# RyanXLi/OneshotDet

Measured on AMD Instinct MI355X. Metric: images/sec/GPU fwd+bwd, 800x1024 target + 127x127 query, bs=8; 1->8 GPU scaling, higher is better.
Workload: dtype bf16; 1 GPU; BASELINE.json configs[2]: bs=8/GPU, 800x1024 target + 127x127 query, bf16 MFMA convs, forward (two R-50-FPN backbones, query pooling, correlation, FCOS head, training proposals) + FCOS loss + backward (stem/layer1 frozen) + gradient all-reduce + SGD(momentum) + weight repack; global_batch=8, parallelism=dp1: one rank, no collective anywhere in the step, world_size=1

## Files before the change

oneshotdet_amd/build.py:

```python
import os
import subprocess
import sys

HERE = os.path.dirname(os.path.abspath(__file__))
CSRC = os.path.join(HERE, "csrc")
LIBDIR = os.path.join(HERE, "lib")
TAG = os.environ.get("OSD_BUILD_TAG", "")
LIB = os.path.join(LIBDIR, "liboneshotdet_hip%s.so" % ("_" + TAG if TAG else ""))
SOURCES = ["osd_error.hip", "conv_igemm.hip", "conv_igemm_dma.hip", "conv_igemm_sp.hip", "conv_pred.hip", "conv_px.hip", "conv_wgrad.hip", "conv_wgrad_sk.hip", "backward.hip", "groupnorm_onepass.hip", "loss.hip", "elementwise.hip", "proposals.hip", "box_head.hip", "transforms.hip", "box_train.hip", "evaluation.hip", "query_avgpool.hip"]
HIPCC = os.environ.get("HIPCC", "/opt/rocm/bin/hipcc")
FLAGS = ["--offload-arch=gfx950", "-O3", "-fPIC", "-std=c++17", "-Wno-unused-result"] + os.environ.get("OSD_BUILD_FLAGS", "").split()


def _stale(target, deps):
    if not os.path.exists(target):
        return True
    t = os.path.getmtime(target)
    return any(os.path.getmtime(d) > t for d in deps)


def build_library(force=False, verbose=True):
    os.makedirs(LIBDIR, exist_ok=True)
    objdir = os.path.join(LIBDIR, "obj" + ("_" + TAG if TAG else ""))
    os.makedirs(objdir, exist_ok=True)
    headers = sorted(os.path.join(CSRC, f) for f in os.listdir(CSRC) if f.endswith(".h")) + [os.path.join(os.path.dirname(HERE), "include", h) for h in ("oneshotdet_hip.h", "oneshotdet_hip_box_modes.h", "oneshotdet_hip_soft_labels.h")]
    keep = set(src.replace(".hip", ".o") for src in SOURCES)
    for f in os.listdir(objdir):
        if f.endswith(".o") and f not in keep:
            os.remove(os.path.join(objdir, f))
    objs, procs = [], []
    for src in SOURCES:
        s = os.path.join(CSRC, src)
        o = os.path.join(objdir, src.replace(".hip", ".o"))
        objs.append(o)
        if force or _stale(o, [s] + headers):
            cmd = [HIPCC] + FLAGS + ["-c", s, "-o", o]
            if verbose:
                print(" ".join(cmd), flush=True)
            procs.append((src, subprocess.Popen(cmd, stdout=subprocess.PIPE, stderr=subprocess.STDOUT)))
    for src, p in procs:
        out, _ = p.communicate()
        if p.returncode != 0:
            sys.stderr.write(out.decode())
            raise RuntimeError("hipcc failed on %s" % src)
    if force or procs or _stale(LIB, objs):
        cmd = [HIPCC, "--offload-arch=gfx950", "-shared", "-fPIC", "-o", LIB] + objs
        if verbose:
            print(" ".join(cmd), flush=True)
        subprocess.check_call(cmd)
    return LIB


if __name__ == "__main__":
    print(build_library(force="--force" in sys.argv))
```

oneshotdet_amd/csrc/conv_wgrad.hip:

```cpp
#include "wgrad_params.h"

namespace {

__device__ __attribute__((aligned(256))) unsigned g_wzero[64];

__device__ __forceinline__ void wg_dma16(const void* gsrc, unsigned lds_dst) {
  unsigned keep;
  asm volatile(
      "s_mov_b32 %0, m0\n\ts_mov_b32 m0, %2\n\ts_nop 0\n\tglobal_load_lds_dwordx4 %1, off\n\ts_mov_b32 m0, %0"
      : "=&s"(keep)
      : "v"(gsrc), "s"(lds_dst)
      : "memory");
}

template <typename T, int BKP, int NST, int WCO, int WCI, int WM, int WN, bool ILV = false>
__global__ void __launch_bounds__(64 * WM * WN, (WM * WN == 4 && WCO + WCI == 3) ? 2 : 1) conv_wgrad_kernel(WgradParams gp) {
  constexpr int NW = WM * WN;
  constexpr int EPC = 16 / (int)sizeof(T);
  constexpr int TWS = 256 / (int)sizeof(T);
  constexpr int TCO = WCO * TWS, TCI = WCI * TWS;
  constexpr int OPB = BKP * 256;
  constexpr int STAGE = (WCO + WCI) * OPB;
  constexpr int PPS = BKP / 4;
  constexpr int IPA = WCO * PPS / NW;
// ... 717 lines not shown
#pragma unroll
          for (int k = 0; k < 4; ++k) red[((co * 9 + t) * 4 + k) * 64 + lane] = acc[co][t][k];
    }
    __syncthreads();
    if (wave == 0) {
#pragma unroll
      for (int co = 0; co < 4; ++co)
#pragma unroll
        for (int t = 0; t < 9; ++t)
#pragma unroll
          for (int k = 0; k < 4; ++k) acc[co][t][k] += red[((co * 9 + t) * 4 + k) * 64 + lane];
    }
    __syncthreads();
  }
  if (wave == 0) {
    float* pp = part + ((size_t)blockIdx.x * gridDim.y + cg) * 36 * 256 + lane * 4;
#pragma unroll
    for (int co = 0; co < 4; ++co)
#pragma unroll
      for (int t = 0; t < 9; ++t)
        *reinterpret_cast<f32x4*>(pp + (co * 9 + t) * 256) = f32x4{acc[co][t][0], acc[co][t][1], acc[co][t][2], acc[co][t][3]};
  }
  if (cg == 0) {
    if (lane == 4) {
#pragma unroll
      for (int co = 0; co < 4; ++co) part_b[((size_t)blockIdx.x * 4 + wave) * 4 + co] = bsum[co];
    }
  }
}

__global__ void pred_wgrad_reduce_kernel(const float* __restrict__ part, const float* __restrict__ part_b, float* __restrict__ dw,
                                         float* __restrict__ db, int blocks, int groups, int C, int cout) {
  const int i = blockIdx.x * blockDim.x + threadIdx.x;
  const int n = cout * 9 * C;
  const int per = (blocks + gridDim.y - 1) / gridDim.y;
  const int b0 = blockIdx.y * per, b1 = min(blocks, b0 + per);
  if (i < n) {
    const int c = i % C, ct = i / C;
    const int cg = c >> 8, cl = c & 255;
    const size_t stride = (size_t)groups * 36 * 256;
    const float* p = part + ((size_t)cg * 36 + ct) * 256 + cl;
    float s0 = 0.f, s1 = 0.f, s2 = 0.f, s3 = 0.f;
    int b = b0;
    for (; b + 3 < b1; b += 4) {
      s0 += p[(size_t)b * stride]; s1 += p[(size_t)(b + 1) * stride]; s2 += p[(size_t)(b + 2) * stride]; s3 += p[(size_t)(b + 3) * stride];
    }
    for (; b < b1; ++b) s0 += p[(size_t)b * stride];
    if (b0 < b1) atomicAdd(dw + i, (s0 + s1) + (s2 + s3));
  } else if (db != nullptr && i < n + cout) {
    const int co = i - n;
    float s = 0.f;
    for (int b = b0 * 4; b < b1 * 4; ++b) s += part_b[(size_t)b * 4 + co];
    if (b0 < b1) atomicAdd(db + co, s);
  }
}

template <typename T>
__global__ void __launch_bounds__(256) bias_grad_kernel(const T* __restrict__ dy, float* __restrict__ db, int M, int C,
                                                        int stride, int rows_per_block) {
  const int c = blockIdx.y * blockDim.x + threadIdx.x;
  const int p_lo = blockIdx.x * rows_per_block, p_hi = min(M, p_lo + rows_per_block);
  if (c >= C || p_lo >= p_hi) return;
  float s = 0.f;
  for (int m = p_lo; m < p_hi; ++m) s += to_f32(dy[(size_t)m * stride + c]);
  atomicAdd(db + c, s);
}

}

#define OSD_STREAM(s) reinterpret_cast<hipStream_t>(s)

extern "C" int osd_bias_grad(const void* dy, float* db, int m, int c, int stride, int dtype, void* stream);

static bool wgrad_dense_input(const osd_conv_desc* d) {
  return d->in_stride_w == d->cin && d->in_stride_h == d->w * d->cin && (long long)d->in_stride_n == (long long)d->h * d->w * d->cin;
}

struct WgradProblem {
  const osd_conv_desc* d;
  int n, h, w;
  const void* x; const void* dy; const float* scale; float* dw; float* db;
};

static int wgrad_xr_launch(int n_seg, const WgradProblem* pr, hipStream_t s) {
  if (n_seg < 1 || n_seg > kMaxSeg) return osd_fail(OSD_ERR_INVALID_ARG, "wgrad: 1..%d segments", kMaxSeg);
  const osd_conv_desc* d0 = pr[0].d;
  static const int kTargets[8] = {512, 256, 128, 64, 1024, 768, 1536, 2048};
  const int a = d0->algo - 1 - 128;
  const int x = a & 15, target = kTargets[(a >> 4) & 7];
  if (a < 0 || a >= 128 || x > 2) return osd_fail(OSD_ERR_INVALID_ARG, "wgrad: unknown algo %d", d0->algo);
  const int bkp = x == 1 ? 64 : 32;
  WgradParams p;
  p.n_seg = n_seg;
  p.sk_units = 0;
  long long work = 0;
  for (int i = 0; i < n_seg; ++i) {
    const osd_conv_desc* d = pr[i].d;
    WgradSeg& g = p.seg[i];
    g.owner = 0;
    const int h = pr[i].h, w = pr[i].w;
    if (d->dtype != OSD_BF16 || d->r != 3 || d->s != 3 || d->stride_h != 1 || d->stride_w != 1 || d->pad_h != 1 || d->pad_w != 1 ||
        d->cout % 128 || d->cin % 128 || d->out_stride % 8 || !(w % bkp == 0 || bkp % w == 0))
      return osd_fail(OSD_ERR_UNSUPPORTED, "wgrad (filter-row kernel): bf16 3x3 / 1 / 1, channels in 128s, width %d vs %d-pixel stages", w, bkp);
    const long long M = (long long)pr[i].n * h * w;
    if (M <= 0 || M > 0x7fffffffLL || !pr[i].x || !pr[i].dy || !pr[i].dw) return osd_fail(OSD_ERR_INVALID_ARG, "wgrad: bad segment %d", i);
    if (M * d->cin > 0x7fffffffLL) return osd_fail(OSD_ERR_UNSUPPORTED, "wgrad: input of segment %d has more than 2^31 elements", i);
    g.x = pr[i].x; g.dy = pr[i].dy; g.dw = pr[i].dw; g.scale = pr[i].scale; g.db = pr[i].db;
    g.H = h; g.W = w; g.Ho = h; g.Wo = w; g.M = (int)M;
    g.Cin = d->cin; g.Cout = d->cout; g.R = 3; g.S = 3; g.sh = g.sw = 1; g.ph = g.pw = 1;
    g.dy_stride = d->out_stride; g.Ktot = 9 * d->cin;
    g.tilesCo = d->cout / 128; g.tilesCi = d->cin / 128;
    work += M * g.tilesCo * g.tilesCi * 3;
  }
  long long rows = (work + target - 1) / target;
  rows = (rows + 63) / 64 * 64;
  if (rows < 128) rows = 128;
  long long nblocks = 0;
  for (int i = 0; i < n_seg; ++i) {
    WgradSeg& g = p.seg[i];
    int sp = (int)((g.M + rows - 1) / rows);
    if (sp < 1) sp = 1;
    g.rows_per_split = cdiv(cdiv(g.M, sp), 64) * 64;
    const int splits = cdiv(g.M, g.rows_per_split);
    g.block_begin = (int)nblocks;
    nblocks += (long long)g.tilesCo * g.tilesCi * 3 * splits;
    if (nblocks > 0x7fffffffLL) return osd_fail(OSD_ERR_INVALID_ARG, "wgrad: bad grid");
  }
  for (int i = n_seg; i < kMaxSeg; ++i) p.seg[i] = p.seg[0];
  p.n_blocks = (int)nblocks;
  p.partials = nullptr;
#define OSD_WGX(BK, NS)                                                                                               \
  do {                                                                                                                \
    auto kern = conv_wgrad_xr_kernel<BK, NS>;                                                                         \
    constexpr int lds = NS * (BK + BK + 4) * 256;                                                                     \
    static bool attr = false;                                                                                         \
    if (!attr) { (void)hipFuncSetAttribute(reinterpret_cast<const void*>(kern), hipFuncAttributeMaxDynamicSharedMemorySize, lds); attr = true; } \
    hipLaunchKernelGGL(kern, dim3((unsigned)nblocks), dim3(512), lds, s, p);                                         \
  } while (0)
  if (x == 0) OSD_WGX(32, 6);
  else if (x == 1) OSD_WGX(64, 4);
  else OSD_WGX(32, 8);
#undef OSD_WGX
  return osd_check_launch("conv_wgrad_xr");
}

static int wgrad_launch_v(int n_seg, const WgradProblem* pr, hipStream_t s, int variant_override);
static int wgrad_launch(int n_seg, const WgradProblem* pr, hipStream_t s) {
  int rc = wgrad_launch_v(n_seg, pr, s, -1);
  if (rc == OSD_ERR_UNSUPPORTED && n_seg >= 1 && pr[0].d->algo == 0) rc = wgrad_launch_v(n_seg, pr, s, 0);
  return rc;
}

static int wgrad_launch_v(int n_seg, const WgradProblem* pr, hipStream_t s, int variant_override) {
  if (n_seg < 1 || n_seg > kMaxSeg) return osd_fail(OSD_ERR_INVALID_ARG, "wgrad: 1..%d segments", kMaxSeg);
  const osd_conv_desc* d0 = pr[0].d;
  if (d0->algo > 128) return wgrad_xr_launch(n_seg, pr, s);
  static int env_target = -1, env_variant = -1;
  if (env_target < 0) { const char* e = getenv("OSD_WGRAD_BLOCKS"); env_target = e ? atoi(e) : 512; }
  if (env_variant < 0) { const char* e = getenv("OSD_WGRAD_VARIANT"); env_variant = e ? atoi(e) : 0; }
  static const int kTargets[8] = {512, 256, 128, 64, 1024, 768, 1536, 2048};
  int target = env_target, variant = variant_override >= 0 ? variant_override : env_variant, code = 0;
  if (d0->algo > 0) {
    const int a = d0->algo - 1;
    if (a >= 128) return osd_fail(OSD_ERR_INVALID_ARG, "wgrad: unknown algo %d", d0->algo);
    variant = a & 15;
    code = a >> 4;
    target = kTargets[code];
  }
  if (d0->dtype == OSD_F32) target *= 8;
  const bool bf = d0->dtype == OSD_BF16;
  if (!bf && variant != 0) variant = 0;
  const int sub_co = bf && (variant == 3 || variant == 4 || variant == 5 || variant == 7 || variant == 8 || variant == 9 || variant == 11 || variant == 13 || variant == 14) ? 2 : 1;
// ... 459 lines not shown
```

oneshotdet_amd/csrc/wgrad_params.h:

```cpp
#pragma once
#include "osd_common.h"
#include <cstddef>

constexpr int kMaxSeg = 24;

struct WgradSeg {
  const void* x;
  const void* dy;
  float* dw;
  const float* scale;
  float* db;
  int H, W, Ho, Wo, M, rows_per_split;
  int Cin, Cout, R, S, sh, sw, ph, pw, dy_stride, tilesCo, tilesCi, Ktot;
  int block_begin;
  int stage_begin;
  int owner;
};

struct WgradParams {
  WgradSeg seg[kMaxSeg];
  int n_seg;
  int n_blocks;
  int sk_units;
  int sk_teams;
  int sk_total;
  float* partials;
};

typedef __attribute__((address_space(1))) float wg_gfloat;
__device__ __forceinline__ void wg_atomic_add(float* ptr, float v) {
  (void)__hip_atomic_fetch_add((wg_gfloat*)ptr, v, __ATOMIC_RELAXED, __HIP_MEMORY_SCOPE_AGENT);
}

template <int TA, int TB>
__device__ __forceinline__ void wg_owner_add(float* base, int Ktot, const f32x4 (&acc)[TA][TB], const float (&scv)[TA][4]) {
#pragma unroll
  for (int i = 0; i < TA; ++i) {
    float old[4][TB];
#pragma unroll
    for (int e = 0; e < 4; ++e)
#pragma unroll
      for (int j = 0; j < TB; ++j) old[e][j] = ((const wg_gfloat*)(base + (size_t)(i * 16 + e) * Ktot))[j * 16];
#pragma unroll
    for (int e = 0; e < 4; ++e)
#pragma unroll
      for (int j = 0; j < TB; ++j) ((wg_gfloat*)(base + (size_t)(i * 16 + e) * Ktot))[j * 16] = old[e][j] + acc[i][j][e] * scv[i][e];
    __builtin_amdgcn_sched_barrier(0);
  }
}

template <int N> __device__ __forceinline__ void wg_wait_vmcnt() { asm volatile("s_waitcnt vmcnt(%0)" ::"n"(N) : "memory"); }


template <typename T> __device__ __forceinline__ int wg_swz(int row) {
  if constexpr (sizeof(T) == 2) return 2 * (row & 7);
  else return 4 * (row & 3);
}

int osd_wgrad_sk_launch(const WgradParams& p, hipStream_t s);
```

oneshotdet_amd/ops.py:

```python
import ctypes as C
import os

import torch

from . import _lib, spec
from ._lib import (ACT_EXP_SCALE, ACT_NONE, ACT_RELU, GN_SPLITS, OSD_BF16, OSD_F32, RES_DOWN2X, RES_NONE, RES_SAME, RES_UP2X,
                   ConvDesc)

__all__ = ["ACT_NONE", "ACT_RELU", "ACT_EXP_SCALE", "RES_NONE", "RES_SAME", "RES_UP2X", "RES_DOWN2X"]


from . import streams

_stream_handle = streams.raw_handle


def _stream():
    return C.c_void_p(_stream_handle())


from .trace import rec as _rec


def _dt(t):
# ... 20 lines not shown
def _chk_dev(*ts):
    for t in ts:
        if t is not None and not t.is_cuda:
            raise _lib.OsdError("oneshotdet_amd ops need device tensors (no CPU path): got %s" % t.device)


def conv_out(n, k, s, p):
    return (n + 2 * p - k) // s + 1


class PackedConv(object):
    __slots__ = ("w", "bias", "cout", "cout_store", "w_rows", "cin_k", "cin_real", "r", "s", "stem")

    def __init__(self, w, bias, cout, cout_store, w_rows, cin_k, r, s, stem=False, cin_real=None):
        self.w, self.bias, self.cout, self.cout_store = w, bias, cout, cout_store
        self.w_rows, self.cin_k, self.r, self.s, self.stem = w_rows, cin_k, r, s, stem
        self.cin_real = cin_k if cin_real is None else cin_real


def _round_up(x, m):
    return (x + m - 1) // m * m


def pack_conv(weight, bias=None, bn=None, dtype=torch.float32, stem=False):
    _chk_dev(weight)
    cout, cin, r, s = weight.shape
    weight = weight.contiguous().float()
    scale = None
    if bn is not None:
        g, b, mean, var = (t.float() for t in bn)
        scale = (g * var.rsqrt()).contiguous()
        fbias = b - mean * scale
    else:
        fbias = bias.float() if bias is not None else torch.zeros(cout, device=weight.device)
    cout_store = _round_up(cout, 4)
    w_rows = _round_up(cout, 16)
    bias_p = torch.zeros(_round_up(cout_store, 16), device=weight.device, dtype=torch.float32)
    bias_p[:cout] = fbias
    if stem:
        assert (cin, r, s) == (3, 7, 7)
        wp = torch.empty((w_rows, 7, 32), device=weight.device, dtype=dtype)
        _lib.call("osd_pack_stem_weight", _p(weight), _p(scale), _p(wp), cout, w_rows, _dt(wp), _stream())
        return PackedConv(wp, bias_p, cout, cout_store, w_rows, 32, 7, 1, stem=True, cin_real=3)
    mult = 64 if dtype == torch.bfloat16 else 16
    cin_pad = _round_up(cin, mult)
    wp = torch.empty((w_rows, r, s, cin_pad), device=weight.device, dtype=dtype)
    _lib.call("osd_pack_conv_weight", _p(weight), _p(scale), _p(wp), cout, cin, r, s, w_rows, cin_pad, _dt(wp),
              _stream())
    return PackedConv(wp, bias_p, cout, cout_store, w_rows, cin_pad, r, s, cin_real=cin)


def pack_image(images, dtype, hp, wp, pad_t=3, pad_l=3):
    _chk_dev(images)
    n, c, h, w = images.shape
    assert c == 3 and images.dtype == torch.float32
    out = torch.empty((n, hp, wp, 4), device=images.device, dtype=dtype)
    _lib.call("osd_pack_image", _ptr(images.contiguous()), _p(out), n, h, w, hp, wp, pad_t, pad_l, _dt(out), _stream())
    _rec("pack_image", x=images, out=out, pad_t=pad_t, pad_l=pad_l)
    return out


class PackedImages(object):

    def __init__(self, tensor, hw, image_sizes):
        self.tensor, self.hw, self.image_sizes = tensor, tuple(hw), [tuple(s) for s in image_sizes]

    @property
    def shape(self):
        return (self.tensor.shape[0], 3, self.hw[0], self.hw[1])


def stem_input(images, dtype):
    n, _, h, w = images.shape
    ho, wo = conv_out(h, 7, 2, 3), conv_out(w, 7, 2, 3)
    if isinstance(images, PackedImages):
        assert images.tensor.dtype == dtype, "PackedImages were written as %s, the engine computes in %s" % (images.tensor.dtype, dtype)
        return images.tensor, (ho, wo)
    hp, wp = max(2 * (ho - 1) + 7, h + 3), max(2 * (wo - 1) + 8, w + 3)
    wp += wp & 1
    return pack_image(images, dtype, hp, wp), (ho, wo)


from .tuner import (TUNE_LOG, refine_in_step, wgrad_timer, ALGO_CACHE, CONV_ALGO_PX, CONV_ALGO_PX_WIDE, SPLIT_CACHE, WGRAD_ALGO_CACHE, _TUNING, _candidate_runs, _photo_finish, _time_launches, _tune, _tune_wgrad,
                    conv_algo_candidates, replaying, tuning, wgrad_algo_candidates, wgrad_xr_candidates)


class ConvSrc2(C.Structure):
    _fields_ = [("x", C.c_void_p), ("w2", C.c_void_p), ("cin2", C.c_int32), ("h", C.c_int32), ("w", C.c_int32),
                ("stride", C.c_int32)]


def conv2d(x, pc, stride=1, pad=0, act=ACT_NONE, res=None, res_mode=RES_NONE, relu_in=False, act_scale=1.0, out=None,
           out_hw=None, algo=None, mask=None, act_scale_dev=None, x2=None, x2_stride=1, pc2=None, bias=None):
    _chk_dev(x, res, out)
    if x2 is not None:
        return _conv2d_two_sources(x, x2, x2_stride, pc, act, out, algo, pc2, bias)
    shape = x.shape
    okey = None if out is None else out.shape[-1]
    ckey = (shape, x.dtype, pc.cout_store, pc.w_rows, pc.cin_k, pc.r, pc.s, pc.stem, stride, pad, act, res_mode,
            None if res is None else res.shape, bool(relu_in), float(act_scale), mask is not None, out_hw, okey)
    ent = _CONV_DESCS.get(ckey)
    if ent is None:
        ent = _CONV_DESCS[ckey] = _build_conv_desc(x, pc, stride, pad, act, res, res_mode, relu_in, act_scale, out, out_hw, mask)
    d, oshape, key = ent[0], ent[1], ent[2]
    if out is None:
        out = torch.empty(oshape, device=x.device, dtype=x.dtype)
    if mask is not None:
        assert mask.shape == out.shape and mask.dtype == out.dtype
    args = (_p(x), _p(pc.w), _p(pc.bias), _p(res), _p(mask), _p(act_scale_dev), None, _p(out), _stream())
    if algo is None:
        algo = ALGO_CACHE.get(key)
        if algo is None:
            algo = _tune(key, d, lambda: _lib.call("osd_conv2d_fwd", C.byref(d), *args), prewarm=lambda: x.float().sum()) if _TUNING[0] else 0
    d.algo = algo
    try:
        _lib.call("osd_conv2d_fwd", C.byref(d), *args)
    except _lib.OsdError as e:
        if getattr(e, "code", 0) != -2 or algo == 0 or ALGO_CACHE.get(key) != algo:
            raise
        del ALGO_CACHE[key]
        d.algo = 0
        _lib.call("osd_conv2d_fwd", C.byref(d), *args)
    _rec("conv", x=x, w=pc.w, bias=pc.bias, cout=pc.cout_store, r=pc.r, s=pc.s, stem=pc.stem, stride=stride, pad=pad, act=act,
         res=res, res_mode=res_mode, relu_in=bool(relu_in), act_scale=float(act_scale), act_scale_dev=act_scale_dev, mask=mask,
         out=out, algo=d.algo, key=key)
    return out


_CONV_DESCS = {}


def _p(t):
    return None if t is None else t.data_ptr()


def _build_conv_desc(x, pc, stride, pad, act, res, res_mode, relu_in, act_scale, out, out_hw, mask):
    n, h, w, c = x.shape
    d = ConvDesc()
    d.dtype = _dt(x)
    d.n, d.h, d.w = n, h, w
    if pc.stem:
        ho, wo = out_hw
        d.cin, d.r, d.s = 32, 7, 1
        d.in_stride_n, d.in_stride_h, d.in_stride_w = h * w * 4, w * 4, 4
        d.stride_h, d.stride_w, d.pad_h, d.pad_w = 2, 2, 0, 0
        d.h, d.w = h, w - 7
        assert 2 * (wo - 1) + 8 <= w and 2 * (ho - 1) + 7 <= h, "stem input not padded enough"
    else:
        assert c == pc.cin_k, "input channels %d != packed K per tap %d" % (c, pc.cin_k)
        ho, wo = conv_out(h, pc.r, stride, pad), conv_out(w, pc.s, stride, pad)
        d.cin, d.r, d.s = c, pc.r, pc.s
        d.in_stride_n, d.in_stride_h, d.in_stride_w = h * w * c, w * c, c
        d.stride_h = d.stride_w = stride
        d.pad_h = d.pad_w = pad
    d.ho, d.wo, d.cout, d.w_rows = ho, wo, pc.cout_store, pc.w_rows
    oshape = (n, ho, wo, pc.cout_store)
    d.out_stride = pc.cout_store if out is None else out.shape[-1]
    d.res_mode = res_mode
    if res_mode != RES_NONE:
        d.res_h, d.res_w, d.res_stride = res.shape[1], res.shape[2], res.shape[3]
        if res_mode == RES_UP2X:
            assert res.shape[1] * 2 == ho and res.shape[2] * 2 == wo, "top-down map must be exactly half size"
        if res_mode == RES_DOWN2X:
            assert res.shape[1] >= 2 * ho - 1 and res.shape[2] >= 2 * wo - 1, "the every-other-pixel addend must cover the output"
    d.act, d.act_scale, d.relu_in = act, float(act_scale), int(relu_in)
    key = (d.dtype, n, ho, wo, d.cout, d.cin, d.r, d.s, d.stride_h, d.pad_h, res_mode, act, int(relu_in), mask is not None)
    return (d, oshape, key)
# ... 1118 lines not shown
```

oneshotdet_amd/tuner.py:

```python
import os

import torch

from . import _lib
from ._lib import OSD_BF16

class _Cache(dict):
    census = False

    def __init__(self, *a, **kw):
        dict.__init__(self, *a, **kw)
        self.hits = {}

    def get(self, key, default=None):
        if self.census:
            self.hits[key] = self.hits.get(key, 0) + 1
        return dict.get(self, key, default)


SPLIT_CACHE = _Cache()
WGRAD_ALGO_CACHE = _Cache()
TUNE_LOG = {"ALGO_CACHE": {}, "WGRAD_ALGO_CACHE": {}, "SPLIT_CACHE": {}}

ALGO_CACHE = _Cache()
# ... 81 lines not shown


_FLUSH = [None]


def _time_launches_cold(fn, prewarm=None):
    if _REPLAY[0]:
        raise RuntimeError("tuner cache miss while replaying another rank's choices: this rank met a shape the tuning rank did not")
    if _FLUSH[0] is None:
        _FLUSH[0] = torch.zeros(128 * 1024 * 1024, device="cuda")
    reps = max(3, int(os.environ.get("OSD_TUNE_REPS", "3")))
    total = 0.0
    for _ in range(reps):
        _FLUSH[0].add_(1.0)
        if prewarm is not None:
            prewarm()
        ev = [torch.cuda.Event(enable_timing=True) for _ in range(2)]
        ev[0].record()
        fn()
        ev[1].record()
        torch.cuda.synchronize()
        total += ev[0].elapsed_time(ev[1])
    return total / reps


def release_tuning_scratch():
    _FLUSH[0] = None


def _photo_finish(timed, retime):
    timed = sorted(timed)
    if not timed:
        return 0
    margin = 1.0 + float(os.environ.get("OSD_TUNE_MARGIN", "0.05"))
    close = [(t, a) for t, a in timed if t <= timed[0][0] * margin][:3]
    if len(close) < 2:
        return timed[0][1]
    best = {a: t for t, a in close}
    for _ in range(2):
        for _, a in close:
            best[a] = min(best[a], retime(a))
    return min(best.items(), key=lambda kv: kv[1])[0]


def _tune(key, d, launch, cands=None, prewarm=None):
    timed = []
    pixels = d.n * d.ho * d.wo
    cold = 0 < pixels <= COLD_MAX_PIXELS and d.cout > 16 and not os.environ.get("OSD_TUNE_WARM_ONLY")
    time_it = (lambda f: _time_launches_cold(f, prewarm)) if cold else _time_launches
    forced = os.environ.get("OSD_FORCE_ALGO_3X3_256")
    if forced and d.cout == 256 and d.r == 3 and d.stride_h == 1:
        d.algo = int(forced)
        try:
            launch()
            torch.cuda.synchronize()
            ALGO_CACHE[key] = int(forced)
            return int(forced)
        except _lib.OsdError:
            pass
    for algo in (cands if cands is not None else conv_algo_candidates(d.cout, d.relu_in, has_mask=bool(key[-1]), pixels=pixels if pixels > 0 else None)):
        d.algo = algo
        try:
            launch()
        except _lib.OsdError:
            continue
        timed.append((time_it(launch), algo))

    def retime(algo):
        d.algo = algo
        return time_it(launch)
    best = _photo_finish(timed, retime)
    ALGO_CACHE[key] = best
    TUNE_LOG["ALGO_CACHE"][key] = sorted(timed)
    return best


def wgrad_xr_candidates(dtype, cout, cin, r, s, stride, pad, widths):
    if dtype != OSD_BF16 or (r, s, stride, pad) != (3, 3, 1, 1) or cout % 128 or cin % 128 or not widths:
        return []
    xs = [x for x, bk in ((0, 32), (1, 64), (2, 32)) if all(w % bk == 0 or bk % w == 0 for w in widths)]
    return [1 + 128 + x + 16 * t for t in (0, 1, 2, 4, 5, 6, 7) for x in xs]


def wgrad_algo_candidates(dtype, cout=0, cin=0):
    variants = [0, 1, 2] if dtype == OSD_BF16 else [0]
    if dtype == OSD_BF16:
        variants.append(15)
    if dtype == OSD_BF16 and cout >= 256 and cin >= 256:
        variants += [3, 4, 5, 8, 9, 13]
    if dtype == OSD_BF16 and cin >= 256:
        variants += [6, 10]
    if dtype == OSD_BF16 and cout >= 256:
        variants += [7, 11, 14]
    excl = [int(v) for v in os.environ.get("OSD_WGRAD_EXCLUDE", "").split(",") if v]
    variants = [v for v in variants if v not in excl]
    return [1 + v + 16 * t for t in (0, 1, 2, 3, 4, 5, 6, 7) for v in variants if not (v == 3 and t > 3)]


def _candidate_runs(fn):
    try:
        fn()
        return True
    except _lib.OsdError as e:
        if getattr(e, "code", 0) == -2:
            return False
        raise


def wgrad_timer():
    return _time_launches_cold if os.environ.get("OSD_TUNE_WGRAD_COLD") else _time_launches


def _tune_wgrad(key, d, launch, dw, db, widths=None):
    _time_launches = wgrad_timer()
    sdw = torch.empty_like(dw)
    sdb = None if db is None else torch.empty_like(db)
    timed = []
    cands = wgrad_algo_candidates(d.dtype, d.cout, d.cin)
    if os.environ.get("OSD_WGRAD_XR"):
        cands = cands + wgrad_xr_candidates(d.dtype, d.cout, d.cin, d.r, d.s, d.stride_h, d.pad_h, widths)
    verbose = os.environ.get("OSD_TUNE_VERBOSE")
    for algo in cands:
        d.algo = algo
        if not _candidate_runs(lambda: launch(sdw, sdb)):
            if verbose:
                print("   wgrad tuner: variant %d code %d refused" % ((algo - 1) & 15, (algo - 1) >> 4))
            continue
        t = _time_launches(lambda: launch(sdw, sdb))
        if verbose:
            print("   wgrad tuner: variant %d code %d  %.1f us" % ((algo - 1) & 15, (algo - 1) >> 4, t * 1e3))
        timed.append((t, algo))

    def retime(algo):
        d.algo = algo
        return _time_launches(lambda: launch(sdw, sdb))
    best = _photo_finish(timed, retime)
    WGRAD_ALGO_CACHE[key] = best
    TUNE_LOG["WGRAD_ALGO_CACHE"][key] = sorted(timed)
    return best


def refine_in_step(step, sync, n_steps=12, margin=0.10, min_share=0.004, gain=0.003, budget_s=100.0, verbose=False, cycle=1):
    import time
    caches = {"ALGO_CACHE": ALGO_CACHE, "WGRAD_ALGO_CACHE": WGRAD_ALGO_CACHE, "SPLIT_CACHE": SPLIT_CACHE}

    n_steps = (n_steps + cycle - 1) // cycle * cycle

    def measure():
        evs = []
        for _ in range(cycle):
            step()
        for _ in range(n_steps):
            e = torch.cuda.Event(enable_timing=True)
            e.record()
            evs.append(e)
            step()
        e = torch.cuda.Event(enable_timing=True)
        e.record()
        evs.append(e)
        sync()
        ms = sorted(a.elapsed_time(b) for a, b in zip(evs[:-1], evs[1:]))
        return ms[len(ms) // 2] if cycle == 1 else sum(ms) / len(ms)

    for c in caches.values():
        c.hits = {}
        c.census = True
    try:
        step()
        sync()
    finally:
        for c in caches.values():
            c.census = False
    step_ms = measure()
    todo = []
    for name, cache in caches.items():
        for key, hits in cache.hits.items():
            log = TUNE_LOG[name].get(key)
            if not log or key not in cache:
                continue
            cur = cache[key]
            t_cur = min([t for t, a in log if a == cur] or [log[0][0]])
            share = hits * t_cur / step_ms
            alts = [a for t, a in log if a != cur and t <= t_cur * (1.0 + margin)][:2]
            if share >= min_share and alts:
                todo.append((share, name, key, alts))
    todo.sort(key=lambda t: -t[0])
    t0, changed = time.time(), []
    for share, name, key, alts in todo:
        cache = caches[name]
        for alt in alts:
            if time.time() - t0 > budget_s:
                break
            base = cache[key]
            a1 = measure()
            cache[key] = alt
            b1 = measure()
            cache[key] = base
            a2 = measure()
            cache[key] = alt
            b2 = measure()
            keep = b1 < a1 * (1.0 - gain) and b2 < a2 * (1.0 - gain)
            if verbose:
                print("   refine %s share %.3f: %s -> %s  %.3f/%.3f  %.3f/%.3f ms  %s" % (name, share, base, alt, a1, b1, a2, b2, "KEEP" if keep else "-"), flush=True)
# ... 6 lines not shown
```

Before: 785.8 images/sec.

## Add pipelined filter-row wgrad kernel as tuner candidate for multi-level convs

```diff
diff --git a/oneshotdet_amd/build.py b/oneshotdet_amd/build.py
--- a/oneshotdet_amd/build.py
+++ b/oneshotdet_amd/build.py
@@ -7,7 +7,7 @@
 LIBDIR = os.path.join(HERE, "lib")
 TAG = os.environ.get("OSD_BUILD_TAG", "")
 LIB = os.path.join(LIBDIR, "liboneshotdet_hip%s.so" % ("_" + TAG if TAG else ""))
-SOURCES = ["osd_error.hip", "conv_igemm.hip", "conv_igemm_dma.hip", "conv_igemm_sp.hip", "conv_pred.hip", "conv_px.hip", "conv_wgrad.hip", "conv_wgrad_sk.hip", "backward.hip", "groupnorm_onepass.hip", "loss.hip", "elementwise.hip", "proposals.hip", "box_head.hip", "transforms.hip", "box_train.hip", "evaluation.hip", "query_avgpool.hip"]
+SOURCES = ["osd_error.hip", "conv_igemm.hip", "conv_igemm_dma.hip", "conv_igemm_sp.hip", "conv_pred.hip", "conv_px.hip", "conv_wgrad.hip", "conv_wgrad_sk.hip", "conv_wgrad_fr.hip", "backward.hip", "groupnorm_onepass.hip", "loss.hip", "elementwise.hip", "proposals.hip", "box_head.hip", "transforms.hip", "box_train.hip", "evaluation.hip", "query_avgpool.hip"]
 HIPCC = os.environ.get("HIPCC", "/opt/rocm/bin/hipcc")
 FLAGS = ["--offload-arch=gfx950", "-O3", "-fPIC", "-std=c++17", "-Wno-unused-result"] + os.environ.get("OSD_BUILD_FLAGS", "").split()
 
diff --git a/oneshotdet_amd/csrc/conv_wgrad.hip b/oneshotdet_amd/csrc/conv_wgrad.hip
--- a/oneshotdet_amd/csrc/conv_wgrad.hip
+++ b/oneshotdet_amd/csrc/conv_wgrad.hip
@@ -823,12 +823,67 @@
   const void* x; const void* dy; const float* scale; float* dw; float* db;
 };
 
+static int wgrad_fr_launch(int n_seg, const WgradProblem* pr, hipStream_t s, int code) {
+  const osd_conv_desc* d0 = pr[0].d;
+  if (code > 3) return osd_fail(OSD_ERR_UNSUPPORTED, "wgrad (pipelined filter-row kernel): team mode knows target codes 0..3 (rounds)");
+  if (d0->ordered_ws != nullptr)
+    return osd_fail(OSD_ERR_UNSUPPORTED, "wgrad (pipelined filter-row kernel): team mode adds its partial tiles atomically (not for ordered mode)");
+  WgradParams p;
+  p.n_seg = n_seg;
+  long long total = 0;
+  for (int i = 0; i < n_seg; ++i) {
+    const osd_conv_desc* d = pr[i].d;
+    WgradSeg& g = p.seg[i];
+    const int h = pr[i].h, w = pr[i].w;
+    if (d->dtype != OSD_BF16 || d->r != 3 || d->s != 3 || d->stride_h != 1 || d->stride_w != 1 || d->pad_h != 1 || d->pad_w != 1 ||
+        d->cout % 128 || d->cin % 128 || d->out_stride % 8 || w < 1 || !(w % 64 == 0 || 64 % w == 0))
+      return osd_fail(OSD_ERR_UNSUPPORTED, "wgrad (pipelined filter-row kernel): bf16 3x3 / 1 / 1, channels in 128s, width %d vs 64-pixel stages", w);
+    if (d->cout != d0->cout || d->cin != d0->cin)
+      return osd_fail(OSD_ERR_UNSUPPORTED, "wgrad (pipelined filter-row kernel): team mode needs segments of one conv shape (segment %d differs)", i);
+    const long long M = (long long)pr[i].n * h * w;
+    if (M <= 0 || M > 0x7fffffffLL || !pr[i].x || !pr[i].dy || !pr[i].dw) return osd_fail(OSD_ERR_INVALID_ARG, "wgrad: bad segment %d", i);
+    if ((M + 1024) * d->cin * 2 >= 0x7fffffffLL || (M + 1024) * d->out_stride * 2 >= 0x7fffffffLL)
+      return osd_fail(OSD_ERR_UNSUPPORTED, "wgrad (pipelined filter-row kernel): operands below 2 GiB (segment %d)", i);
+    g.x = pr[i].x; g.dy = pr[i].dy; g.dw = pr[i].dw; g.scale = pr[i].scale; g.db = pr[i].db;
+    g.H = h; g.W = w; g.Ho = h; g.Wo = w; g.M = (int)M;
+    g.Cin = d->cin; g.Cout = d->cout; g.R = 3; g.S = 3; g.sh = g.sw = 1; g.ph = g.pw = 1;
+    g.dy_stride = d->out_stride; g.Ktot = 9 * d->cin;
+    g.tilesCo = d->cout / 128; g.tilesCi = d->cin / 128;
+    g.rows_per_split = 0; g.block_begin = 0; g.owner = 0;
+    g.stage_begin = (int)total;
+    total += M / (w < 64 ? w : 64);
+    if (total > 0x7fffffffLL) return osd_fail(OSD_ERR_INVALID_ARG, "wgrad: bad grid");
+  }
+  static int cus = 0, ring = 0;
+  if (cus == 0) {
+    int dev = 0;
+    if (hipGetDevice(&dev) != hipSuccess || hipDeviceGetAttribute(&cus, hipDeviceAttributeMultiprocessorCount, dev) != hipSuccess || cus < 1) cus = 256;
+    const char* e = getenv("OSD_WGRAD_TEAM_CUS");
+    if (e && atoi(e) > 0) cus = atoi(e);
+    e = getenv("OSD_WGRAD_FR_RING");
+    ring = e ? atoi(e) : 0;
+    if (ring < 2 || ring > 4) ring = 2;
+  }
+  const int units = p.seg[0].tilesCo * p.seg[0].tilesCi * 3;
+  long long teams = (long long)cus * (code + 1) / units;
+  if (teams < 1) return osd_fail(OSD_ERR_UNSUPPORTED, "wgrad (pipelined filter-row kernel): team mode needs at most one output tile x filter row per CU (%d)", units);
+  if (teams > total) teams = total;
+  p.sk_units = units; p.sk_teams = (int)teams; p.sk_total = (int)total;
+  for (int i = n_seg; i < kMaxSeg; ++i) p.seg[i] = p.seg[0];
+  p.n_blocks = (int)(teams * units);
+  p.partials = nullptr;
+  const int rc = osd_wgrad_fr_launch(p, ring, s);
+  if (rc) return rc;
+  return osd_check_launch("conv_wgrad_fr");
+}
+
 static int wgrad_xr_launch(int n_seg, const WgradProblem* pr, hipStream_t s) {
   if (n_seg < 1 || n_seg > kMaxSeg) return osd_fail(OSD_ERR_INVALID_ARG, "wgrad: 1..%d segments", kMaxSeg);
   const osd_conv_desc* d0 = pr[0].d;
   static const int kTargets[8] = {512, 256, 128, 64, 1024, 768, 1536, 2048};
   const int a = d0->algo - 1 - 128;
   const int x = a & 15, target = kTargets[(a >> 4) & 7];
+  if (a >= 0 && a < 128 && x == 3) return wgrad_fr_launch(n_seg, pr, s, a >> 4);
   if (a < 0 || a >= 128 || x > 2) return osd_fail(OSD_ERR_INVALID_ARG, "wgrad: unknown algo %d", d0->algo);
   const int bkp = x == 1 ? 64 : 32;
   WgradParams p;
diff --git a/oneshotdet_amd/csrc/conv_wgrad_fr.hip b/oneshotdet_amd/csrc/conv_wgrad_fr.hip
--- /dev/null
+++ b/oneshotdet_amd/csrc/conv_wgrad_fr.hip
@@ -0,0 +1,284 @@
+#include "wgrad_params.h"
+#include <type_traits>
+
+namespace {
+
+constexpr int NW = 8, WN = 4, TA = 4, TB = 2;
+constexpr int BKP = 64, XR = BKP + 4;
+constexpr int XOFF = BKP * 256, STAGE = (BKP + XR) * 256;
+constexpr int AP = BKP / 4, BP = XR / 4;
+constexpr int LPS = AP / NW + BP / NW;
+static_assert(AP == 2 * NW && BP == 2 * NW + 1, "two dY and two X pieces per wave; the one surplus X piece belongs to wave 0");
+typedef __bf16 T;
+typedef int fr_i32x4 __attribute__((ext_vector_type(4)));
+constexpr unsigned OOB = 0x80000000u;
+
+__device__ __forceinline__ fr_i32x4 fr_make_rsrc(const void* base, unsigned bytes) {
+  const unsigned long long a = (unsigned long long)base;
+  fr_i32x4 r;
+  r[0] = __builtin_amdgcn_readfirstlane((int)(unsigned)a);
+  r[1] = __builtin_amdgcn_readfirstlane((int)((unsigned)(a >> 32) & 0xffffu));
+  r[2] = __builtin_amdgcn_readfirstlane((int)bytes);
+  r[3] = 0x00020000;
+  return r;
+}
+
+__device__ __forceinline__ void fr_dma16(fr_i32x4 rsrc, unsigned voff, unsigned lds_dst) {
+  unsigned keep;
+  asm volatile("s_mov_b32 %0, m0\n\ts_mov_b32 m0, %2\n\ts_nop 0\n\tbuffer_load_dwordx4 %1, %3, 0 offen lds\n\ts_mov_b32 m0, %0"
+               : "=&s"(keep)
+               : "v"(voff), "s"(__builtin_amdgcn_readfirstlane((int)lds_dst)), "s"(rsrc)
+               : "memory");
+}
+
+template <int NST>
+__global__ void __launch_bounds__(64 * NW, 1) conv_wgrad_fr_kernel(WgradParams gp) {
+  extern __shared__ __attribute__((aligned(1024))) char smem[];
+  const unsigned lds0 = (unsigned)(size_t)smem;
+  const int tid = threadIdx.x, lane = tid & 63;
+  const int wave = __builtin_amdgcn_readfirstlane(tid >> 6);
+  const int wm = wave / WN, wn = wave % WN;
+
+  int bid;
+  {
+    const int nb = gridDim.x, b = blockIdx.x;
+    const int q = nb >> 3, r = nb & 7, xcd = b & 7, idx = b >> 3;
+    bid = (xcd < r ? xcd * (q + 1) : r * (q + 1) + (xcd - r) * q) + idx;
+  }
+  typedef const __attribute__((address_space(4))) char* kptr;
+  typedef unsigned long long u64;
+  const kptr seg0 = (kptr)__builtin_amdgcn_kernarg_segment_ptr() + offsetof(WgradParams, seg);
+#define OSD_KSEG(idx, type, field) (*reinterpret_cast<const __attribute__((address_space(4))) type*>(seg0 + (idx) * (int)sizeof(WgradSeg) + offsetof(WgradSeg, field)))
+
+  const int tm = bid / gp.sk_units, unit = bid - tm * gp.sk_units;
+  const int g0 = (int)((long long)tm * gp.sk_total / gp.sk_teams);
+  const int g1 = (int)((long long)(tm + 1) * gp.sk_total / gp.sk_teams);
+  int sidx = 0;
+  for (int i = 1; i < gp.n_seg; ++i)
+    if (g0 >= OSD_KSEG(i, int, stage_begin)) sidx = i;
+
+  typedef __attribute__((ext_vector_type(4))) __bf16 bf4;
+  typedef __attribute__((address_space(3))) bf4* lds_bf4_ptr;
+  const int g = lane >> 4, t16 = lane & 15, q4 = t16 >> 2, pp = t16 & 3;
+  const int h8 = (pp & 1) * 8;
+  const int rr = 4 * g + q4;
+  const int a_c0 = wm * 64, b_c0 = wn * 32;
+  const unsigned fa0 = rr * 256 + ((((a_c0 >> 3) + (pp >> 1)) ^ wg_swz<T>(rr)) << 4) + h8;
+  unsigned fb0[3];
+#pragma unroll
+  for (int s = 0; s < 3; ++s) fb0[s] = XOFF + (rr + s) * 256 + ((((b_c0 >> 3) + (pp >> 1)) ^ wg_swz<T>(rr + s)) << 4) + h8;
+  auto read_frag = [&](unsigned stage_base, unsigned f0, int idx, int k32) -> bf16x8 {
+    const unsigned a = ((stage_base + f0) ^ (unsigned)(idx << 5)) + (unsigned)(k32 * 32 * 256);
+    const bf4 lo = __builtin_amdgcn_ds_read_tr16_b64_v4bf16((lds_bf4_ptr)a);
+    const bf4 hi = __builtin_amdgcn_ds_read_tr16_b64_v4bf16((lds_bf4_ptr)(a + 16 * 256));
+    bf16x8 v;
+#pragma unroll
+    for (int e = 0; e < 4; ++e) { v[e] = lo[e]; v[e + 4] = hi[e]; }
+    return v;
+  };
+  const int plrow = lane >> 4, plpos = lane & 15;
+  const int r0 = 4 * wave + plrow;
+  const int sw_chunk = plpos ^ wg_swz<T>(r0);
+
+  f32x4 acc[3][TA][TB];
+#pragma unroll
+  for (int s = 0; s < 3; ++s)
+#pragma unroll
+    for (int i = 0; i < TA; ++i)
+#pragma unroll
+      for (int j = 0; j < TB; ++j) acc[s][i][j] = f32x4{0.f, 0.f, 0.f, 0.f};
+  float bsum = 0.f;
+
+  for (;;) {
+    const kptr sb = seg0 + sidx * (int)sizeof(WgradSeg);
+#define OSD_WSEG(type, field) (*reinterpret_cast<const __attribute__((address_space(4))) type*>(sb + offsetof(WgradSeg, field)))
+    const void* px = (const void*)OSD_WSEG(u64, x);
+    const void* pdy = (const void*)OSD_WSEG(u64, dy);
+    float* pdw = (float*)OSD_WSEG(u64, dw);
+    const float* pscale = (const float*)OSD_WSEG(u64, scale);
+    float* pdb = (float*)OSD_WSEG(u64, db);
+    const int H = OSD_WSEG(int, H), W = OSD_WSEG(int, W), M = OSD_WSEG(int, M), Cin = OSD_WSEG(int, Cin);
+    const int dy_stride = OSD_WSEG(int, dy_stride), tilesCo = OSD_WSEG(int, tilesCo), tilesCi = OSD_WSEG(int, tilesCi);
+    const int Ktot = OSD_WSEG(int, Ktot), sbeg = OSD_WSEG(int, stage_begin);
+#undef OSD_WSEG
+    const int co_tile = unit % tilesCo, nt = unit / tilesCo;
+    const int fr = nt / tilesCi, ci_tile = nt % tilesCi;
+    const int co0 = co_tile * 128, ci0 = ci_tile * 128;
+    const int SP = W < BKP ? W : BKP;
+    const int kts = M / SP;
+    const int t_lo = max(g0, sbeg) - sbeg, t_hi = min(g1, sbeg + kts) - sbeg;
+    const bool last = g1 <= sbeg + kts || sidx + 1 >= gp.n_seg;
+    const int KT = t_hi - t_lo;
+
+    if (KT > 0) {
+      const fr_i32x4 dyrs = fr_make_rsrc(pdy, (unsigned)M * (unsigned)dy_stride * 2u);
+      const fr_i32x4 xrs = fr_make_rsrc(px, (unsigned)M * (unsigned)Cin * 2u);
+      const unsigned pa = (unsigned)(r0 * dy_stride + co0 + sw_chunk * 8) * 2u;
+      const int cb = ci0 + sw_chunk * 8;
+      const int xoff = (fr - 1) * W - 1;
+      int nx_left = KT, nx_m = t_lo * SP, nx_ho, nx_wo;
+      {
+        const int row = nx_m / W;
+        nx_wo = nx_m - row * W;
+        nx_ho = row % H;
+      }
+      auto issue_piece = [&](int pc, unsigned st) {
+        const bool sv = nx_left > 0;
+        if (pc < 2) {
+          const bool ok = sv && r0 + 32 * pc < SP;
+          const unsigned off = pa + (unsigned)((nx_m + 32 * pc) * dy_stride) * 2u;
+          fr_dma16(dyrs, ok ? off : OOB, st + (unsigned)((wave + 8 * pc) * 1024));
+        } else {
+          const int i = pc - 2;
+          const int j = r0 + 32 * i;
+          const bool ok = sv && (unsigned)(nx_ho - 1 + fr) < (unsigned)H && j < SP + 2 && (unsigned)(nx_wo - 1 + j) < (unsigned)W;
+          const unsigned off = (unsigned)((nx_m + xoff + j) * Cin + cb) * 2u;
+          fr_dma16(xrs, ok ? off : OOB, st + (unsigned)(XOFF + (wave + 8 * i) * 1024));
+        }
+      };
+      auto next_stage = [&]() {
+        --nx_left;
+        nx_m += SP;
+        nx_wo += SP;
+        if (nx_wo >= W) { nx_wo = 0; if (++nx_ho >= H) nx_ho = 0; }
+      };
+      const bool do_bias = pdb != nullptr;
+      const int nslots = 3 * tilesCi;
+      int bias_turn = (t_lo % nslots + nslots - nt) % nslots;
+      auto bias_stage = [&](int buf) {
+        const int cc = tid & 127, row0 = (tid >> 7) * (BKP / 4);
+        const char* sa = smem + buf * STAGE + row0 * 256 + (cc % 8) * (int)sizeof(T);
+        const int chunk = cc / 8;
+#pragma unroll
+        for (int i = 0; i < BKP / 4; ++i)
+          bsum += to_f32(*reinterpret_cast<const T*>(sa + i * 256 + ((chunk ^ wg_swz<T>(i)) << 4)));
+      };
+
+      bf16x8 af[TA], xf[3][TB];
+      auto k_step = [&](unsigned cst, auto ck_tag, unsigned nst, auto nk_tag, auto bar_tag, unsigned dst) {
+        constexpr int ck = decltype(ck_tag)::value, nk = decltype(nk_tag)::value;
+        constexpr bool BAR = decltype(bar_tag)::value;
+#pragma unroll
+        for (int j = 0; j < TB; ++j) xf[2][j] = read_frag(cst, fb0[2], j, ck);
+#pragma unroll
+        for (int s = 0; s < 3; ++s) {
+#pragma unroll
+          for (int i = 0; i < TA; ++i) {
+            const int grp = s * TA + i;
+#pragma unroll
+            for (int j = 0; j < TB; ++j) acc[s][i][j] = __builtin_amdgcn_mfma_f32_16x16x32_bf16(af[i], xf[s][j], acc[s][i][j], 0, 0, 0);
+            if constexpr (BAR) {
+              if (grp == 1) {
+                __builtin_amdgcn_sched_barrier(0);
+                asm volatile("s_waitcnt lgkmcnt(0)" ::: "memory");
+                if (wave == 0) wg_wait_vmcnt<(NST - 2) * (LPS + 1)>();
+                else wg_wait_vmcnt<(NST - 2) * LPS>();
+                __builtin_amdgcn_s_barrier();
+              }
+              if (grp >= 2 && grp < 2 + LPS) issue_piece(grp - 2, dst);
+              if (grp == 2 + LPS && wave == 0) issue_piece(LPS, dst);
+            }
+            if (grp == TA) {
+#pragma unroll
+              for (int j = 0; j < TB; ++j) xf[0][j] = read_frag(nst, fb0[0], j, nk);
+            }
+            if (grp == 2 * TA) {
+#pragma unroll
+              for (int j = 0; j < TB; ++j) xf[1][j] = read_frag(nst, fb0[1], j, nk);
+            }
+            if (s == 2) af[i] = read_frag(nst, fa0, i, nk);
+            __builtin_amdgcn_sched_barrier(0);
+          }
+        }
+      };
+      using K0 = std::integral_constant<int, 0>;
+      using K1 = std::integral_constant<int, 1>;
+      __builtin_amdgcn_s_barrier();
+#pragma unroll
+      for (int st = 0; st < NST; ++st) {
+#pragma unroll
+        for (int pc = 0; pc < LPS; ++pc) issue_piece(pc, lds0 + st * STAGE);
+        if (wave == 0) issue_piece(LPS, lds0 + st * STAGE);
+        next_stage();
+      }
+      if (wave == 0) wg_wait_vmcnt<(NST - 1) * (LPS + 1)>();
+      else wg_wait_vmcnt<(NST - 1) * LPS>();
+      __builtin_amdgcn_s_barrier();
+#pragma unroll
+      for (int i = 0; i < TA; ++i) af[i] = read_frag(lds0, fa0, i, 0);
+#pragma unroll
+      for (int s = 0; s < 2; ++s)
+#pragma unroll
+        for (int j = 0; j < TB; ++j) xf[s][j] = read_frag(lds0, fb0[s], j, 0);
+      int cur = 0;
+      for (int kt = 0; kt < KT; ++kt) {
+        const int nxt = cur + 1 == NST ? 0 : cur + 1;
+        const unsigned cst = lds0 + cur * STAGE, nst = lds0 + nxt * STAGE;
+        if (do_bias && bias_turn == 0) bias_stage(cur);
+        bias_turn = bias_turn + 1 == nslots ? 0 : bias_turn + 1;
+        k_step(cst, K0(), cst, K1(), std::false_type(), 0u);
+        k_step(cst, K1(), nst, K0(), std::true_type(), cst);
+        next_stage();
+        cur = nxt;
+      }
+      wg_wait_vmcnt<0>();
+    }
+
+    bool flush = last;
+    if (!last) {
+      flush = (float*)OSD_KSEG(sidx + 1, u64, dw) != pdw || (const float*)OSD_KSEG(sidx + 1, u64, scale) != pscale ||
+              (float*)OSD_KSEG(sidx + 1, u64, db) != pdb;
+    }
+    if (flush) {
+      if (pdb != nullptr) wg_atomic_add(pdb + co0 + (tid & 127), bsum);
+      const int co_w = co0 + wm * 64 + (lane >> 4) * 4;
+      const int ci_w = ci0 + wn * 32 + (lane & 15);
+      float scv[TA][4];
+#pragma unroll
+      for (int i = 0; i < TA; ++i)
+#pragma unroll
+        for (int e = 0; e < 4; ++e) scv[i][e] = pscale ? pscale[co_w + i * 16 + e] : 1.f;
+#pragma unroll
+      for (int s = 0; s < 3; ++s) {
+        float* base = pdw + (size_t)co_w * Ktot + (fr * 3 + s) * Cin + ci_w;
+#pragma unroll
+        for (int i = 0; i < TA; ++i)
+#pragma unroll
+          for (int e = 0; e < 4; ++e) {
+            float* row = base + (size_t)(i * 16 + e) * Ktot;
+#pragma unroll
+            for (int j = 0; j < TB; ++j) wg_atomic_add(row + j * 16, acc[s][i][j][e] * scv[i][e]);
+          }
+      }
+      if (last) return;
+#pragma unroll
+      for (int s = 0; s < 3; ++s)
+#pragma unroll
+        for (int i = 0; i < TA; ++i)
+#pragma unroll
+          for (int j = 0; j < TB; ++j) acc[s][i][j] = f32x4{0.f, 0.f, 0.f, 0.f};
+      bsum = 0.f;
+    }
+    ++sidx;
+  }
+#undef OSD_KSEG
+}
+
+template <int NST> void fr_launch(const WgradParams& p, hipStream_t s) {
+  constexpr int lds = NST * STAGE;
+  static bool attr = false;
+  if (!attr) {
+    (void)hipFuncSetAttribute(reinterpret_cast<const void*>(conv_wgrad_fr_kernel<NST>), hipFuncAttributeMaxDynamicSharedMemorySize, lds);
+    attr = true;
+  }
+  hipLaunchKernelGGL((conv_wgrad_fr_kernel<NST>), dim3((unsigned)p.n_blocks), dim3(64 * NW), lds, s, p);
+}
+
+}
+
+int osd_wgrad_fr_launch(const WgradParams& p, int ring, hipStream_t s) {
+  if (ring == 2) fr_launch<2>(p, s);
+  else if (ring == 3) fr_launch<3>(p, s);
+  else fr_launch<4>(p, s);
+  return 0;
+}
diff --git a/oneshotdet_amd/csrc/wgrad_params.h b/oneshotdet_amd/csrc/wgrad_params.h
--- a/oneshotdet_amd/csrc/wgrad_params.h
+++ b/oneshotdet_amd/csrc/wgrad_params.h
@@ -58,3 +58,5 @@
 }
 
 int osd_wgrad_sk_launch(const WgradParams& p, hipStream_t s);
+
+int osd_wgrad_fr_launch(const WgradParams& p, int ring, hipStream_t s);
diff --git a/oneshotdet_amd/ops.py b/oneshotdet_amd/ops.py
--- a/oneshotdet_amd/ops.py
+++ b/oneshotdet_amd/ops.py
@@ -126,7 +126,7 @@
 
 
 from .tuner import (TUNE_LOG, refine_in_step, wgrad_timer, ALGO_CACHE, CONV_ALGO_PX, CONV_ALGO_PX_WIDE, SPLIT_CACHE, WGRAD_ALGO_CACHE, _TUNING, _candidate_runs, _photo_finish, _time_launches, _tune, _tune_wgrad,
-                    conv_algo_candidates, replaying, tuning, wgrad_algo_candidates, wgrad_xr_candidates)
+                    conv_algo_candidates, replaying, tuning, wgrad_algo_candidates, wgrad_fr_candidates, wgrad_xr_candidates)
 
 
 class ConvSrc2(C.Structure):
diff --git a/oneshotdet_amd/tuner.py b/oneshotdet_amd/tuner.py
--- a/oneshotdet_amd/tuner.py
+++ b/oneshotdet_amd/tuner.py
@@ -187,6 +187,17 @@
     return [1 + 128 + x + 16 * t for t in (0, 1, 2, 4, 5, 6, 7) for x in xs]
 
 
+WGRAD_FR_STAGE = 64
+
+
+def wgrad_fr_candidates(dtype, cout, cin, r, s, stride, pad, widths):
+    if dtype != OSD_BF16 or (r, s, stride, pad) != (3, 3, 1, 1) or cout % 128 or cin % 128 or not widths:
+        return []
+    if not all(w > 0 and (w % WGRAD_FR_STAGE == 0 or WGRAD_FR_STAGE % w == 0) for w in widths):
+        return []
+    return [1 + 128 + 3 + 16 * t for t in (0, 1, 2, 3)]
+
+
 def wgrad_algo_candidates(dtype, cout=0, cin=0):
     variants = [0, 1, 2] if dtype == OSD_BF16 else [0]
     if dtype == OSD_BF16:
@@ -216,14 +227,25 @@
     return _time_launches_cold if os.environ.get("OSD_TUNE_WGRAD_COLD") else _time_launches
 
 
+def _wgrad_key_is_multi_level(key):
+    return key[0] == "multi" or (len(key) > 1 and isinstance(key[1], tuple) and len(key[1]) > 0 and isinstance(key[1][0], tuple))
+
+
+def _wgrad_tune_candidates(key, d, widths):
+    cands = wgrad_algo_candidates(d.dtype, d.cout, d.cin)
+    if os.environ.get("OSD_WGRAD_XR"):
+        cands = cands + wgrad_xr_candidates(d.dtype, d.cout, d.cin, d.r, d.s, d.stride_h, d.pad_h, widths)
+    if _wgrad_key_is_multi_level(key) and not os.environ.get("OSD_NO_WGRAD_FR"):
+        cands = cands + wgrad_fr_candidates(d.dtype, d.cout, d.cin, d.r, d.s, d.stride_h, d.pad_h, widths)
+    return cands
+
+
 def _tune_wgrad(key, d, launch, dw, db, widths=None):
     _time_launches = wgrad_timer()
     sdw = torch.empty_like(dw)
     sdb = None if db is None else torch.empty_like(db)
     timed = []
-    cands = wgrad_algo_candidates(d.dtype, d.cout, d.cin)
-    if os.environ.get("OSD_WGRAD_XR"):
-        cands = cands + wgrad_xr_candidates(d.dtype, d.cout, d.cin, d.r, d.s, d.stride_h, d.pad_h, widths)
+    cands = _wgrad_tune_candidates(key, d, widths)
     verbose = os.environ.get("OSD_TUNE_VERBOSE")
     for algo in cands:
         d.algo = algo
```

Result: no change. 792.6 images/sec, median of 6 (+0.9%).
